# hgpeterson/nuPGCM

Measured on AMD Instinct MI355X. Metric: timesteps/sec (evolve!+invert! loop; inversion SpMV GB/s in 'roofline'), higher is better.
Workload: dtype f64 arithmetic; fp32-STORED Krylov basis and fp32 gather-layout copy of the SpMV input (the library's default at rtol >= 1e-7; products, sums, x += V y and the restart residual are fp64 - the all-fp64 figure is `fp64_basis`); 1 GPU; bowl3D_h0.02: example parameters of examples/bowl_mixing.jl (eps=0.2, alpha=1/2, mu_rho=1, N2=2, BDF2 dt=0.001), full evolve!+invert! timestep loop; tets=526720, nu=2052199, np=98592, nb=707204, nnz_A=126821881, node_block_storage=True, full_nodes=658911, surface_nodes=37733, gmres_memory=20, gmres_itmax=0, initial_guess=x_{n-1} (the reference's warm start), all_solved=True, preconditioner=Diagonal(scalar=73847.66715287707), parallelism=1 GPU

## Files before the change

### nupgcm_amd/csrc/gmres.hip

```cpp
#include <algorithm>
#include <chrono>
#include <cmath>
#include <cstdlib>
#include <type_traits>

#include <hip/hip_ext.h>

#include "common.h"
#include "spmv_device.h"
#include "spmv_window.h"

namespace npg {

constexpr int kKB = 512;
constexpr int kKP = kPartStride;
constexpr int kNS = kKB / kKP;
constexpr int kMaxG = 768;
constexpr int kMaxI = kMaxG / kNS;
constexpr int kNormSlot = kKP - 1;
constexpr int kMaxRows = 2048;

struct Snap {
    double eps, rnorm0, rnorm, beta, zeta;
    int iter, inner, done, npass, first, nreorth, pad0, pad1;
// ... 5 lines not shown
};

struct GDev {
    CsrDev A;
    const TileDesc *tile_ptr;
    int ntiles, n, mem;
    int nt_int;
    const WTileDesc *wt_ptr;
    WinDev W;
    int nwt, nwt_int, wl;
    int word;
    int wpre;
    int pkind;
    double pscalar;
    const double *pdiag;
    const double *b;
    double *x, *Vi, *w, *wt;
    double *P1, *P2, *PR;
    int G1, G2, GP1, GP2;
    int GR;
    int split;
    int64_t ldv;
    float *Vf;
    int pyth;
    int lazy2;
    int rev;
    GatherMap xg;
    const int32_t *gslot;
    int fast;
    const double *Q1, *Q2, *QR;
    int nQ1, nQ2, nQR;
    int onefold;
    int vdots;
    int fusedrows;
    struct RowsHandOff *ho;
    Snap *C, *T;
    double *c, *s, *z, *R, *hcol1, *wnorm2;
    double *hist;
    int hist_cap;
    const GParams *prm;
};

__device__ __forceinline__ void sym_givens(double a, double b, double &c, double &s, double &rho) {
    if (b == 0.0) {
        c = (a == 0.0) ? 1.0 : copysign(1.0, a);
        s = 0.0;
        rho = fabs(a);
    } else if (a == 0.0) {
        c = 0.0;
        s = copysign(1.0, b);
        rho = fabs(b);
    } else if (fabs(b) > fabs(a)) {
        const double t = a / b;
        s = copysign(1.0, b) / sqrt(1.0 + t * t);
        c = s * t;
        rho = b / s;
    } else {
        const double t = b / a;
        c = copysign(1.0, a) / sqrt(1.0 + t * t);
        s = c * t;
        rho = a / c;
    }
}

struct KShared {
    double red[kKP];
    double h[kKP], h2[kKP], cc[kKP], ss[kKP], y[kKP];
    Snap T;
    double rho, zcol;
    int fin;
    int reorth;
};

__device__ __forceinline__ void store_partial_row(double acc, double *tmp, double *part) {
    __syncthreads();
    tmp[threadIdx.x] = acc;
    __syncthreads();
    if (threadIdx.x < kKP) {
        double s = 0.0;
#pragma unroll
        for (int sl = 0; sl < kNS; ++sl) s += tmp[sl * kKP + threadIdx.x];
        part[(size_t)blockIdx.x * kKP + threadIdx.x] = s;
    }
}

__device__ void finalize_column(const GDev &d, int colj, KShared &sh, double *tmp) {
    const int t32 = threadIdx.x & (kKP - 1);
    const double h1 = d.hcol1[colj * kKP + t32];
    const double cv = d.c[t32], sv = d.s[t32];
    const Snap prev = d.T[colj];
    const double wnorm2 = d.wnorm2[colj];
    const double q1 = group_sum_dpp<kKP>(t32 <= colj ? h1 * h1 : 0.0);
    const double n2f = wnorm2 - q1;
    const bool need2 = !d.pyth && (!d.lazy2 || !(n2f >= fmax(d.prm->eta2, 1e-4) * wnorm2));
    if (need2) reduce_partials<kNS, kMaxI>(d.Q2, d.nQ2, kKP, tmp, sh.red);
    if (threadIdx.x < kKP) {
        sh.h[threadIdx.x] = h1;
        sh.h2[threadIdx.x] = (need2 && !d.fast && (int)threadIdx.x <= colj) ? sh.red[threadIdx.x] : 0.0;
        sh.cc[threadIdx.x] = cv;
        sh.ss[threadIdx.x] = sv;
    }
    __syncthreads();
    if (threadIdx.x == 0) {
        Snap t = prev;
        sh.fin = (t.done == 0) ? 1 : 0;
        sh.reorth = 0;
        if (t.done == 0) {
            double n2;
            if (d.pyth) {
                n2 = fmax(n2f, 0.0);
                if (n2f < 1e-4 * wnorm2) {
                    t.pad0 += 1;
                    t.done = 5;
                    sh.fin = 0;
                }
            } else if (!need2) {
                n2 = fmax(n2f, 0.0);
            } else {
                n2 = sh.red[kNormSlot];
            }
          if (t.done == 0) {
            const bool due = need2 && n2 < d.prm->eta2 * wnorm2;
            if (due && d.fast) t.pad1 += 1;
            const bool reorth = due && !d.fast;
            if (reorth) {
                double q = 0.0;
                for (int i = 0; i <= colj; ++i) {
// ... 199 lines not shown
            const int rb = r + kNS;
            const bool hb = rb < nr;
            const int rowa = r0 + r, rowb = r0 + (hb ? rb : r);
            double va = (k < j) ? d.Vi[vidx(rowa, k, d.n, d.ldv)] : 0.0;
            double vb = (hb && k < j) ? d.Vi[vidx(rowb, k, d.n, d.ldv)] : 0.0;
            double ta = d.wt[rowa], tb = d.wt[rowb];
            const double wa = sw[r] * inv_beta * precond_row(d, rowa);
            const double wb = hb ? sw[rb] * inv_beta * precond_row(d, rowb) : 0.0;
            if (ro) {
                ta -= group_sum_dpp<kKP>(h2k * va);
                tb -= group_sum_dpp<kKP>(h2k * vb);
            }
            if (k == j) {
                va = ta * inv_beta;
                d.Vi[vidx(rowa, j, d.n, d.ldv)] = va;
                if (hb) {
                    vb = tb * inv_beta;
                    d.Vi[vidx(rowb, j, d.n, d.ldv)] = vb;
                }
            }
            if (k == 0) {
                d.w[rowa] = wa;
                if (hb) d.w[rowb] = wb;
            }
            acc += (k == kNormSlot) ? wa * wa + wb * wb : va * wa + vb * wb;
        }
    }
    if (FUSED) store_partial_row(acc, tmp, d.P1);
}

constexpr int kRB = 256;
constexpr int kMaxRowsI = kMaxG / (kRB / 32);

template <int NG, typename BT>
__device__ __forceinline__ void load_row_cols(const BT *__restrict__ Vi, int64_t row, int64_t ldv, int j,
                                              double (&v)[8 * NG]) {
#pragma unroll
    for (int k = 0; k < 8 * NG; ++k) v[k] = (k <= j) ? (double)Vi[(size_t)k * (size_t)ldv + (size_t)row] : 0.0;
}
template <typename BT>
__device__ __forceinline__ const BT *basis_ptr(const GDev &d);
template <>
__device__ __forceinline__ const double *basis_ptr<double>(const GDev &d) { return d.Vi; }
template <>
__device__ __forceinline__ const float *basis_ptr<float>(const GDev &d) { return d.Vf; }

template <int NG>
__device__ __forceinline__ void store_partial_row_rows(const double (&acc)[8 * NG], double nrm, double *tmp, double *part) {
    const int wave = threadIdx.x >> 6, lane = threadIdx.x & 63;
    __syncthreads();
    if (lane < kKP) tmp[wave * kKP + lane] = 0.0;
    __syncthreads();
#pragma unroll
    for (int k = 0; k < 8 * NG; ++k) {
        const double s = group_sum_dpp<64>(acc[k]);
        if (lane == 0 && k < kNormSlot) tmp[wave * kKP + k] = s;
    }
    const double sn = group_sum_dpp<64>(nrm);
    if (lane == 0) tmp[wave * kKP + kNormSlot] = sn;
    __syncthreads();
    if (threadIdx.x < kKP) {
        double s = 0.0;
#pragma unroll
        for (int w = 0; w < kRB / 64; ++w) s += tmp[w * kKP + threadIdx.x];
        part[(size_t)blockIdx.x * kKP + threadIdx.x] = s;
    }
}

template <int NG>
__device__ __forceinline__ void load_row_pair_cols(const float *__restrict__ Vf, int64_t r0, bool two, int64_t ldv, int j,
                                                   float2 (&v)[8 * NG]) {
#pragma unroll
    for (int k = 0; k < 8 * NG; ++k) {
        float2 f = make_float2(0.f, 0.f);
        if (k <= j) f = *reinterpret_cast<const float2 *>(Vf + (size_t)k * (size_t)ldv + (size_t)r0);
        if (!two) f.y = 0.f;
        v[k] = f;
    }
}
template <int NG, bool VD = false>
struct RowPair {
    float2 v[8 * NG];
    double w0, w1;
    double2 t;
    int64_t r0;
    bool valid, two;
    __device__ __forceinline__ void load(const GDev &d, int64_t blk, int j) {
        r0 = 2 * (blk * kRB + threadIdx.x);
        valid = r0 < d.n;
        two = r0 + 1 < d.n;
        const int64_t rc = valid ? r0 : 0;
        load_row_pair_cols<NG>(d.Vf, rc, two, d.ldv, VD ? j - 1 : j, v);
        const double2 ww = *reinterpret_cast<const double2 *>(d.w + rc);
        if constexpr (VD) t = *reinterpret_cast<const double2 *>(d.wt + rc);
        w0 = valid ? ww.x : 0.0;
        w1 = (valid && two) ? ww.y : 0.0;
    }
};

template <int NG, typename BT, bool VD = false>
__global__ void __launch_bounds__(kRB) k_gmres_dots_rows(GDev d, int j) {
    static_assert(!VD || sizeof(BT) == 4, "the column is formed by the row-pair kernel of the fp32-stored basis");
    __shared__ double tmp[(kRB / 64) * kKP];
    double acc[8 * NG];
#pragma unroll
    for (int k = 0; k < 8 * NG; ++k) acc[k] = 0.0;
    double nrm = 0.0;
    const Snap *Tj = d.T + j;
    if (Tj->done == 0) {
        if constexpr (sizeof(BT) == 4) {
            const int64_t nblk = ((int64_t)d.n + 2 * kRB - 1) / (2 * kRB);
            RowPair<NG, VD> cur, nxt;
            int64_t blk = blockIdx.x;
            if (blk < nblk) cur.load(d, blk, j);
            double inv_beta = 0.0;
            if constexpr (VD) inv_beta = 1.0 / Tj->beta;
            for (; blk < nblk; blk += gridDim.x) {
                const bool more = blk + gridDim.x < nblk;
                if (more) nxt.load(d, blk + gridDim.x, j);
                if constexpr (VD) {
                    float2 vj = make_float2((float)(cur.t.x * inv_beta), (float)(cur.t.y * inv_beta));
                    if (cur.valid) {
                        float *col = d.Vf + (size_t)j * (size_t)d.ldv + (size_t)cur.r0;
                        if (cur.two)
                            *reinterpret_cast<float2 *>(col) = vj;
                        else
                            *col = vj.x;
                    }
                    if (!cur.two) vj.y = 0.f;
#pragma unroll
                    for (int k = 0; k < 8 * NG; ++k)
                        if (k == j) cur.v[k] = vj;
                }
#pragma unroll
                for (int k = 0; k < 8 * NG; ++k) acc[k] += (double)cur.v[k].x * cur.w0 + (double)cur.v[k].y * cur.w1;
                nrm += cur.w0 * cur.w0 + cur.w1 * cur.w1;
                if (more) cur = nxt;
            }
        } else {
            for (int64_t row = blockIdx.x * (int64_t)kRB + threadIdx.x; row < d.n; row += (int64_t)gridDim.x * kRB) {
                double v[8 * NG];
                load_row_cols<NG, BT>(basis_ptr<BT>(d), row, d.ldv, j, v);
                const double wv = d.w[row];
#pragma unroll
                for (int k = 0; k < 8 * NG; ++k) acc[k] += v[k] * wv;
                nrm += wv * wv;
            }
        }
    }
    store_partial_row_rows<NG>(acc, nrm, tmp, d.P1);
}

template <int NG, bool FAST, typename BT>
__global__ void __launch_bounds__(kRB, (NG < 4 || FAST) ? 3 : 2) k_gmres_orth_rows(GDev d, int j) {
    __shared__ double tmp[(kRB / 32) * kKP];
    __shared__ double red[kKP];
    const Snap T = d.T[j];
    if (T.done != 0) {
        if (threadIdx.x < kKP) d.P2[(size_t)blockIdx.x * kKP + threadIdx.x] = 0.0;
        return;
    }
    constexpr bool kPipe = sizeof(BT) == 4 && FAST;
    const int64_t nblk2 = ((int64_t)d.n + 2 * kRB - 1) / (2 * kRB);
    RowPair<kPipe ? NG : 1> cur;
    if constexpr (kPipe) {
        if ((int64_t)blockIdx.x < nblk2) cur.load(d, d.rev ? nblk2 - 1 - blockIdx.x : blockIdx.x, j);
    }
    reduce_partials<kRB / 32, kMaxRowsI>(d.Q1, d.nQ1, kKP, tmp, red);
    double h[8 * NG], acc[8 * NG];
#pragma unroll
    for (int k = 0; k < 8 * NG; ++k) {
        const double hv = (k <= j) ? red[k] : 0.0;
        const unsigned long long b = __double_as_longlong(hv);
        const unsigned lo = __builtin_amdgcn_readfirstlane((unsigned)b), hi = __builtin_amdgcn_readfirstlane((unsigned)(b >> 32));
        h[k] = __longlong_as_double(((unsigned long long)hi << 32) | lo);
        acc[k] = 0.0;
    }
    double nrm = 0.0;
    if (!d.onefold && blockIdx.x == 0 && threadIdx.x < kKP) {
        d.hcol1[j * kKP + threadIdx.x] = ((int)threadIdx.x <= j) ? red[threadIdx.x] : 0.0;
        if (threadIdx.x == 0) d.wnorm2[j] = red[kNormSlot];
    }
    if constexpr (kPipe) {
        const int64_t nblk = nblk2;
        RowPair<NG> nxt;
        for (int64_t blk = blockIdx.x; blk < nblk; blk += gridDim.x) {
            const int64_t nb = blk + gridDim.x;
            const bool more = nb < nblk;
            if (more) nxt.load(d, d.rev ? nblk - 1 - nb : nb, j);
            double p0 = cur.w0, p1 = cur.w1;
#pragma unroll
            for (int k = 0; k < 8 * NG; ++k) {
                p0 -= h[k] * (double)cur.v[k].x;
                p1 -= h[k] * (double)cur.v[k].y;
            }
            if (cur.valid) {
                if (cur.two)
                    *reinterpret_cast<double2 *>(d.wt + cur.r0) = make_double2(p0, p1);
                else
                    d.wt[cur.r0] = p0;
                if (d.xg.p) {
                    d.xg.p[d.xg.pos((int)cur.r0)] = (float)p0;
                    if (cur.two) d.xg.p[d.xg.pos((int)cur.r0 + 1)] = (float)p1;
                }
            } else {
                p0 = 0.0;
                p1 = 0.0;
            }
            if (!cur.two) p1 = 0.0;
            nrm += p0 * p0 + p1 * p1;
            if (more) cur = nxt;
        }
    } else if constexpr (sizeof(BT) == 4) {
        const int64_t nblk = ((int64_t)d.n + 2 * kRB - 1) / (2 * kRB);
        for (int64_t blk = blockIdx.x; blk < nblk; blk += gridDim.x) {
            const int64_t r0 = 2 * ((d.rev ? nblk - 1 - blk : blk) * kRB + threadIdx.x);
            if (r0 >= d.n) continue;
            const bool two = r0 + 1 < d.n;
            float2 v[8 * NG];
            load_row_pair_cols<NG>(d.Vf, r0, two, d.ldv, j, v);
            const double2 ww = *reinterpret_cast<const double2 *>(d.w + r0);
            double p0 = ww.x, p1 = two ? ww.y : 0.0;
#pragma unroll
            for (int k = 0; k < 8 * NG; ++k) {
                p0 -= h[k] * (double)v[k].x;
                p1 -= h[k] * (double)v[k].y;
            }
            if (two)
                *reinterpret_cast<double2 *>(d.wt + r0) = make_double2(p0, p1);
            else
                d.wt[r0] = p0;
            if (!FAST) {
#pragma unroll
// ... 34 lines not shown
            d.P2[(size_t)blockIdx.x * kKP + threadIdx.x] = t;
        }
    }
}

__global__ void __launch_bounds__(kRB) k_gmres_fold_first(GDev d, int j, double *out) {
    constexpr int NS = kRB / 32;
    __shared__ double tmp[NS * kKP];
    const int done = d.T[j].done;
    const int k = threadIdx.x & (kKP - 1), slice = threadIdx.x >> 5;
    const int nrows = d.GP1;
    double v[kMaxRowsI];
#pragma unroll
    for (int i = 0; i < kMaxRowsI; ++i) {
        const int b = slice + NS * i;
        v[i] = d.P1[(size_t)(b < nrows ? b : 0) * kKP + k];
    }
    double s = 0.0;
#pragma unroll
    for (int i = 0; i < kMaxRowsI; ++i) s += (slice + NS * i < nrows) ? v[i] : 0.0;
    tmp[slice * kKP + k] = s;
    __syncthreads();
    if (threadIdx.x < kKP && done == 0) {
        double t = 0.0;
#pragma unroll
        for (int sl = 0; sl < NS; ++sl) t += tmp[sl * kKP + threadIdx.x];
        out[threadIdx.x] = t;
        d.hcol1[j * kKP + threadIdx.x] = ((int)threadIdx.x <= j) ? t : 0.0;
        if (threadIdx.x == kNormSlot) d.wnorm2[j] = t;
    }
}

constexpr int kFusedMaxCols = 16;
constexpr int kHoLine = 16;
constexpr int kHoShards = kRB / 32;
struct RowsHandOff {
    unsigned long long gen[kHoLine];
    unsigned long long top[kHoLine];
    unsigned long long shard[kHoShards][kHoLine];
    unsigned long long status[kHoLine];
    double slice[kHoShards][kKP];
};
constexpr long long kHandOffTicks = 200000000;

template <int C> struct FusedGeom { static constexpr int B = C <= 8 ? 4 : C <= 12 ? 3 : 2, L = C <= 8 ? 2 : 1; };
static_assert(kFusedMaxCols % 4 == 0, "instances come in steps of four columns");

#define NPG_LD_AGENT(p) __hip_atomic_load((p), __ATOMIC_RELAXED, __HIP_MEMORY_SCOPE_AGENT)
#define NPG_ST_AGENT(p, v) __hip_atomic_store((p), (v), __ATOMIC_RELAXED, __HIP_MEMORY_SCOPE_AGENT)

template <int C>
struct RowTrip {
    float2 v[C];
    double w0, w1;
    template <bool VD>
    __device__ __forceinline__ void load(const GDev &d, int64_t blk, int j, double2 &t) {
        const int64_t r0 = 2 * (blk * kRB + threadIdx.x);
        const bool valid = r0 < d.n, two = r0 + 1 < d.n;
        const int64_t rc = valid ? r0 : 0;
        const int jl = VD ? j - 1 : j;
#pragma unroll
        for (int k = 0; k < C; ++k) {
            float2 f = make_float2(0.f, 0.f);
            if (k <= jl) f = *reinterpret_cast<const float2 *>(d.Vf + (size_t)k * (size_t)d.ldv + (size_t)rc);
            if (!two) f.y = 0.f;
            v[k] = f;
        }
        const double2 ww = *reinterpret_cast<const double2 *>(d.w + rc);
        if constexpr (VD) t = *reinterpret_cast<const double2 *>(d.wt + rc);
        w0 = valid ? ww.x : 0.0;
        w1 = (valid && two) ? ww.y : 0.0;
    }
};

template <int C>
__global__ void __launch_bounds__(kRB, 3) k_gmres_rows_fused(GDev d, int j) {
    constexpr int B = FusedGeom<C>::B, L = FusedGeom<C>::L;
    static_assert(kMaxG == kHoShards * kMaxRowsI && kMaxRowsI % kHoShards == 0, "a shard is one slice of the fold");
    __shared__ float2 lds_v[L * C * kRB];
    __shared__ double lds_w[L * 2 * kRB];
    __shared__ double tmp[(kRB / 32) * kKP];
    __shared__ double red[kKP];
    __shared__ int sh_role, sh_ok;
    const int tid = threadIdx.x, wave = tid >> 6, lane = tid & 63;
    const Snap *Tj = d.T + j;
    if (Tj->done != 0) {
        if (tid < kKP) {
            d.P1[(size_t)blockIdx.x * kKP + tid] = 0.0;
            d.P2[(size_t)blockIdx.x * kKP + tid] = 0.0;
        }
        return;
    }
    RowsHandOff *ho = d.ho;
    if (NPG_LD_AGENT(&ho->status[0]) != 0) return;
    unsigned long long E = 0;
    if (tid == 0) E = NPG_LD_AGENT(&ho->gen[0]);
    const int G = gridDim.x;
    const int64_t nblk = ((int64_t)d.n + 2 * kRB - 1) / (2 * kRB);
    const int nt = (int64_t)blockIdx.x < nblk ? (int)((nblk - 1 - blockIdx.x) / G) + 1 : 0;
    const int nreg = nt < B ? nt : B;
    const int nlds = nt - nreg < L ? nt - nreg : L;
    const int ne = nt - nreg - nlds;
    auto blk_of = [&](int t) { return (int64_t)blockIdx.x + (int64_t)t * G; };

    RowTrip<C> buf[B];
    double2 unused;
    double nrm = 0.0;
    {
        double acc[C];
#pragma unroll
        for (int k = 0; k < C; ++k) acc[k] = 0.0;
        double2 tq[B];
        const double inv_beta = 1.0 / Tj->beta;
#pragma unroll
        for (int s = 0; s < B - 1; ++s)
            if (s < nt) buf[s].template load<true>(d, blk_of(s), j, tq[s]);
        for (int base = 0; base < nt; base += B) {
#pragma unroll
            for (int s = 0; s < B; ++s) {
                const int t = base + s;
                if (t < nt) {
                    const int sp = (s + B - 1) % B;
                    if (t + B - 1 < nt) {
                        if (t - 1 >= ne) {
                            const int sl = t - 1 - ne;
#pragma unroll
                            for (int k = 0; k < C; ++k) lds_v[(sl * C + k) * kRB + tid] = buf[sp].v[k];
                            lds_w[(sl * 2 + 0) * kRB + tid] = buf[sp].w0;
                            lds_w[(sl * 2 + 1) * kRB + tid] = buf[sp].w1;
                        }
                        buf[sp].template load<true>(d, blk_of(t + B - 1), j, tq[sp]);
                    }
                    RowTrip<C> &cur = buf[s];
                    const int64_t r0 = 2 * (blk_of(t) * kRB + tid);
                    const bool valid = r0 < d.n, two = r0 + 1 < d.n;
                    float2 vj = make_float2((float)(tq[s].x * inv_beta), (float)(tq[s].y * inv_beta));
                    if (valid) {
                        float *col = d.Vf + (size_t)j * (size_t)d.ldv + (size_t)r0;
                        if (two)
                            *reinterpret_cast<float2 *>(col) = vj;
                        else
                            *col = vj.x;
                    }
                    if (!two) vj.y = 0.f;
#pragma unroll
                    for (int k = 0; k < C; ++k)
                        if (k == j) cur.v[k] = vj;
#pragma unroll
                    for (int k = 0; k < C; ++k) acc[k] += (double)cur.v[k].x * cur.w0 + (double)cur.v[k].y * cur.w1;
                    nrm += cur.w0 * cur.w0 + cur.w1 * cur.w1;
                }
            }
        }
        __syncthreads();
        if (lane < kKP) tmp[wave * kKP + lane] = 0.0;
        __syncthreads();
#pragma unroll
        for (int k = 0; k < C; ++k) {
            const double s = group_sum_dpp<64>(acc[k]);
            if (lane == 0) tmp[wave * kKP + k] = s;
        }
        const double sn = group_sum_dpp<64>(nrm);
        if (lane == 0) tmp[wave * kKP + kNormSlot] = sn;
        __syncthreads();
        if (tid < kKP) {
            double s = 0.0;
#pragma unroll
            for (int w = 0; w < kRB / 64; ++w) s += tmp[w * kKP + tid];
            NPG_ST_AGENT(d.P1 + (size_t)blockIdx.x * kKP + tid, s);
        }
    }

    const int shard = blockIdx.x % kHoShards;
    const int cnt = (G - shard + kHoShards - 1) / kHoShards;
    const int nsh = G < kHoShards ? G : kHoShards;
    if (wave == 0) asm volatile("s_waitcnt vmcnt(0)" ::: "memory");
    if (tid == 0) {
        const unsigned long long old = __hip_atomic_fetch_add(&ho->shard[shard][0], 1ull, __ATOMIC_RELAXED, __HIP_MEMORY_SCOPE_AGENT);
        sh_role = (old + 1 == (E + 1) * (unsigned long long)cnt) ? 1 : 0;
    }
// ... 54 lines not shown
        int ok = 1;
        const long long t0 = wall_clock64();
        while (NPG_LD_AGENT(&ho->gen[0]) < E + 1) {
            __builtin_amdgcn_s_sleep(8);
            if (wall_clock64() - t0 > kHandOffTicks) {
                NPG_ST_AGENT(&ho->status[0], 1ull);
                ok = 0;
                break;
            }
        }
        sh_ok = ok;
    }
    if (wave == 0) {
        __builtin_amdgcn_fence(__ATOMIC_ACQUIRE, "agent");
        asm volatile("s_waitcnt vmcnt(0)" ::: "memory");
    }
    __syncthreads();
    if (!sh_ok) return;
    if (tid < kKP) {
        const unsigned long long bits = NPG_LD_AGENT(reinterpret_cast<const unsigned long long *>(d.Q1) + tid);
        red[tid] = __longlong_as_double(bits);
    }
    __syncthreads();

    double h[C];
#pragma unroll
    for (int k = 0; k < C; ++k) {
        const double hv = (k <= j) ? red[k] : 0.0;
        const unsigned long long b = __double_as_longlong(hv);
        const unsigned lo = __builtin_amdgcn_readfirstlane((unsigned)b), hi = __builtin_amdgcn_readfirstlane((unsigned)(b >> 32));
        h[k] = __longlong_as_double(((unsigned long long)hi << 32) | lo);
    }
    nrm = 0.0;
    auto update = [&](const RowTrip<C> &cur, int t) {
        const int64_t r0 = 2 * (blk_of(t) * kRB + tid);
        const bool valid = r0 < d.n, two = r0 + 1 < d.n;
        double p0 = cur.w0, p1 = cur.w1;
#pragma unroll
        for (int k = 0; k < C; ++k) {
            float vx = cur.v[k].x, vy = cur.v[k].y;
            asm("" : "+v"(vx), "+v"(vy));
            p0 -= h[k] * (double)vx;
            p1 -= h[k] * (double)vy;
        }
        if (valid) {
            if (two)
                *reinterpret_cast<double2 *>(d.wt + r0) = make_double2(p0, p1);
            else
                d.wt[r0] = p0;
            if (d.xg.p) {
                d.xg.p[d.xg.pos((int)r0)] = (float)p0;
                if (two) d.xg.p[d.xg.pos((int)r0 + 1)] = (float)p1;
            }
        } else {
            p0 = 0.0;
            p1 = 0.0;
        }
        if (!two) p1 = 0.0;
        nrm += p0 * p0 + p1 * p1;
    };
    for (int t = 0; t < ne; ++t) {
        update(early, t);
        if (t + 1 < ne) early.template load<false>(d, blk_of(t + 1), j, unused);
    }
#pragma unroll
    for (int sl = 0; sl < L; ++sl) {
        if (sl < nlds) {
#pragma unroll
            for (int k = 0; k < C; ++k) early.v[k] = lds_v[(sl * C + k) * kRB + tid];
            early.w0 = lds_w[(sl * 2 + 0) * kRB + tid];
            early.w1 = lds_w[(sl * 2 + 1) * kRB + tid];
            update(early, ne + sl);
        }
    }
    {
        const int tr = nt - nreg, rot = tr % B;
#pragma unroll
        for (int ro = 0; ro < B; ++ro) {
            if (ro == rot) {
#pragma unroll
                for (int r = 0; r < B; ++r)
                    if (r < nreg) update(buf[(ro + r) % B], tr + r);
            }
        }
    }
    const double sn2 = group_sum_dpp<64>(nrm);
    __syncthreads();
    if (lane == 0) tmp[wave] = sn2;
    __syncthreads();
    if (tid < kKP) {
        double tt = 0.0;
        if (tid == kNormSlot)
            for (int w = 0; w < kRB / 64; ++w) tt += tmp[w];
        d.P2[(size_t)blockIdx.x * kKP + tid] = tt;
    }
}

__global__ void __launch_bounds__(kKB, 6) k_gmres_orth(GDev d, int j) {
    __shared__ KShared sh;
    __shared__ double tmp[kNS * kKP];
    const Snap T = d.T[j];
    reduce_partials<kNS, kMaxI>(d.Q1, d.nQ1, kKP, tmp, sh.red);
    if (T.done != 0) return;
    const int k = threadIdx.x & (kKP - 1), slot = threadIdx.x >> 5;
    if (blockIdx.x == 0 && threadIdx.x < kKP) {
        d.hcol1[j * kKP + threadIdx.x] = ((int)threadIdx.x <= j) ? sh.red[threadIdx.x] : 0.0;
        if (threadIdx.x == 0) d.wnorm2[j] = sh.red[kNormSlot];
    }
    const double hk = (k <= j) ? sh.red[k] : 0.0;
    double acc = 0.0;
    const int64_t stride = (int64_t)gridDim.x * kNS;
    for (int64_t row = (int64_t)blockIdx.x * kNS + slot; row < d.n; row += 2 * stride) {
        const int64_t rowb = row + stride;
        const bool hb = rowb < d.n;
        const double va = (k <= j) ? d.Vi[vidx(row, k, d.n, d.ldv)] : 0.0;
        const double vb = (hb && k <= j) ? d.Vi[vidx(rowb, k, d.n, d.ldv)] : 0.0;
        const double wa = d.w[row];
// ... 126 lines not shown
    double *P1 = nullptr, *P2 = nullptr, *PR = nullptr;
    Snap *C = nullptr, *T = nullptr;
    double *c = nullptr, *s = nullptr, *z = nullptr, *R = nullptr, *hcol1 = nullptr, *wnorm2 = nullptr;
    double *hist = nullptr;
    int hist_cap = 0;
    GParams *prm = nullptr;
    Snap *h_C = nullptr;
    GParams *h_prm = nullptr;
    int64_t hist_len = 0;
    hipGraph_t graph[2] = {nullptr, nullptr};
    hipGraphExec_t exec[2] = {nullptr, nullptr};
    hipEvent_t ev[2] = {nullptr, nullptr};
    GDev key;
    bool have_graph = false;
    bool profile = false;
    bool explicit_norm = false;
    bool safe_mode = false;
    int split_mode = -1;
    int basis_bits = 0;
    int halo_overlap = -1;
    int dist_graph = -1;
    std::vector<hipEvent_t> pev;
    double prof_ms = 0.0;
    int64_t prof_launches = 0;
    int gather32 = -1;
    float *xg = nullptr;
    int64_t xg_len = 0;
    int xg_key[3] = {-1, -1, -1};
    npg_halo *halo = nullptr;
    double *Rg = nullptr;
    int64_t n_ghost = 0;
    RowsHandOff *ho = nullptr;
    unsigned long long *h_ho = nullptr;
    int fused_blocks = -1;
    bool fused_off = false;
    int32_t cfg[kCfgLen] = {};
    bool have_cfg = false;
};

static int fold_rows(npg_gmres *ws, const double *part, int nrows, int slot, hipStream_t st, bool dist) {
    double *out = ws->Rg + slot * kKP;
    if (dist) return fold_allreduce_rows(ws->ctx, part, nrows, out, st);
    hipLaunchKernelGGL(k_reduce_rows, dim3(1), dim3(1024), 0, st, part, nrows, out);
    return NPG_OK;
}

template <int NG, typename BT>
static void launch_rows_bt(const GDev &d, int j, hipStream_t st, bool orth) {
    if (orth && d.fast)
        hipLaunchKernelGGL((k_gmres_orth_rows<NG, true, BT>), dim3(d.GR), dim3(kRB), 0, st, d, j);
    else if (orth)
        hipLaunchKernelGGL((k_gmres_orth_rows<NG, false, BT>), dim3(d.GR), dim3(kRB), 0, st, d, j);
    else
        hipLaunchKernelGGL((k_gmres_dots_rows<NG, BT>), dim3(d.GR), dim3(kRB), 0, st, d, j);
}
template <int NG>
static void launch_rows(const GDev &d, int j, hipStream_t st, bool orth) {
    if (d.Vf && d.vdots && !orth)
        hipLaunchKernelGGL((k_gmres_dots_rows<NG, float, true>), dim3(d.GR), dim3(kRB), 0, st, d, j);
    else if (d.Vf)
        launch_rows_bt<NG, float>(d, j, st, orth);
    else
        launch_rows_bt<NG, double>(d, j, st, orth);
}

static void launch_rows_kernel(const GDev &d, int j, hipStream_t st, bool orth) {
// ... 349 lines not shown
        const int64_t nbr = A->block_rows(), need = 4 * nslots + (A->n - nbr) + 8;
        if (ws->xg_len < need) {
            if (ws->xg) NPG_HIP(hipFree(ws->xg));
            ws->xg = nullptr;
            NPG_HIP(hipMalloc((void **)&ws->xg, (size_t)need * sizeof(float)));
            ws->xg_len = need;
            ws->xg_key[0] = -1;
        }
        if (ws->xg_key[0] != A->nfull || ws->xg_key[1] != A->nsurf || ws->xg_key[2] != (int)A->n) {
            NPG_HIP(hipMemsetAsync(ws->xg, 0, (size_t)ws->xg_len * sizeof(float), st));
            ws->xg_key[0] = A->nfull;
            ws->xg_key[1] = A->nsurf;
            ws->xg_key[2] = (int)A->n;
        }
        d.xg = GatherMap{ws->xg, 3 * A->nfull, A->nfull, (int)nbr, (int)(4 * nslots - nbr)};
        d.gslot = A->wtile_ptr ? A->gslot : nullptr;
        static const int win_env = getenv("NPG_GMRES_WINDOW") ? atoi(getenv("NPG_GMRES_WINDOW")) : 1;
        if (win_env && ws->gather32 != 2 && d.split && A->wtile_ptr && !A->pk9 && nbr > 0) {
            d.wt_ptr = A->wtile_ptr;
            d.W = win_view(A);
            d.nwt = A->nwtiles;
            d.nwt_int = A->nwtiles_interior;
            d.wl = A->wlanes;
            static const int ord_env = getenv("NPG_WIN_ORD") ? atoi(getenv("NPG_WIN_ORD")) : 0;
            static const int pre_env = getenv("NPG_WIN_PRE") ? atoi(getenv("NPG_WIN_PRE")) : 1;
            d.word = ord_env || (A->nwrow_tiles == 0 && A->m > A->block_rows());
            d.wpre = pre_env;
        }
    }
    const char *onefold_env = getenv("NPG_GMRES_ONEFOLD");
    d.onefold = (!dist && d.split && d.fast && !(onefold_env && atoi(onefold_env) == 0)) ? 1 : 0;
    d.vdots = (d.onefold && d.Vf) ? 1 : 0;
    const char *fusedrows_env = getenv("NPG_GMRES_FUSEDROWS");
    if (!dist && d.split && d.fast && d.Vf && !d.rev && !ws->fused_off && !(fusedrows_env && atoi(fusedrows_env) == 0)) {
        if (ws->fused_blocks < 0) ws->fused_blocks = rows_fused_blocks_per_cu();
        if (d.GR <= ctx->num_cu * ws->fused_blocks) {
            if (!ws->ho) {
                NPG_HIP(hipMalloc((void **)&ws->ho, sizeof(RowsHandOff)));
                NPG_HIP(hipMemsetAsync(ws->ho, 0, sizeof(RowsHandOff), st));
                NPG_HIP(hipHostMalloc((void **)&ws->h_ho, 2 * sizeof(unsigned long long), hipHostMallocDefault));
                ws->h_ho[0] = ws->h_ho[1] = 0;
            }
            d.fusedrows = 1;
            d.ho = ws->ho;
            d.onefold = d.vdots = 1;
        }
    }
    if (dist) {
        d.Q1 = ws->Rg;
        d.Q2 = ws->Rg + kKP;
        d.QR = ws->Rg + 2 * kKP;
        d.nQ1 = d.nQ2 = d.nQR = 1;
    } else {
        d.Q1 = d.P1;
        d.Q2 = d.P2;
        d.QR = d.PR;
        d.nQ1 = d.GP1;
        d.nQ2 = d.GP2;
        d.nQR = d.G1;
        if (d.onefold) {
            d.Q1 = ws->Rg;
            d.nQ1 = 1;
        }
    }
    d.C = ws->C;
    d.T = ws->T;
    d.c = ws->c;
    d.s = ws->s;
    d.z = ws->z;
    d.R = ws->R;
    d.hcol1 = ws->hcol1;
    d.wnorm2 = ws->wnorm2;
    d.hist = ws->hist;
    d.hist_cap = ws->hist_cap;
    d.prm = ws->prm;

    if (itmax <= 0) itmax = 2 * ws->n;
    ws->h_prm->atol = atol;
    ws->h_prm->rtol = rtol;
// ... 5 lines not shown
    c0.first = 1;
    ws->h_C[0] = c0;
    NPG_HIP(hipMemcpyAsync(ws->C, ws->h_C, sizeof(Snap), hipMemcpyHostToDevice, st));
    NPG_HIP(hipStreamSynchronize(st));

    static const int traced = getenv("ROCPROFILER_LIBRARY_CTOR") || getenv("ROCPROF_OUTPUT_PATH") || getenv("ROCP_TOOL_LIBRARIES");
    static const int eager = getenv("NPG_GMRES_EAGER") ? atoi(getenv("NPG_GMRES_EAGER")) : traced;
    static bool said = false;
    if (eager && traced && !getenv("NPG_GMRES_EAGER") && !said && (said = true))
        fprintf(stderr, "[npg] rocprofv3 detected: GMRES restart cycles are launched eagerly instead of replayed from hipGraphs "
                        "(rocprofiler-sdk faults on graph launches that wrap the AQL ring; NPG_GMRES_EAGER=0 overrides)\n");
    static const int trace = getenv("NPG_GMRES_TRACE") ? atoi(getenv("NPG_GMRES_TRACE")) : 0;

    static const int dist_graph_env = getenv("NPG_DIST_GRAPH") ? atoi(getenv("NPG_DIST_GRAPH")) : -1;
    const bool kernel_only = dist && comm_is_kernel_only(ws->ctx);
    const bool graph_dist = dist && !ws->ctx->shm &&
                            (kernel_only ? (dist_graph_env != 0 && ws->dist_graph != 0) : ((ws->dist_graph > 0 || dist_graph_env > 0) && ws->ctx->comm));
    auto capture_graphs = [&]() -> int {
        for (int k = 0; k < 2; ++k) {
            if (ws->exec[k]) hipGraphExecDestroy(ws->exec[k]);
            if (ws->graph[k]) hipGraphDestroy(ws->graph[k]);
            ws->exec[k] = nullptr;
            ws->graph[k] = nullptr;
            ws->have_graph = false;
            NPG_HIP(hipStreamBeginCapture(st, hipStreamCaptureModeThreadLocal));
            int rcg = launch_cycle(d, A->lanes, st, nullptr, ws, dist != nullptr);
            if (rcg) {
                hipGraph_t broken = nullptr;
                hipStreamEndCapture(st, &broken);
                if (broken) hipGraphDestroy(broken);
                return rcg;
            }
            NPG_HIP(hipMemcpyAsync(ws->h_C + k, ws->C, sizeof(Snap), hipMemcpyDeviceToHost, st));
            if (d.fusedrows) NPG_HIP(hipMemcpyAsync(ws->h_ho + k, d.ho->status, sizeof(unsigned long long), hipMemcpyDeviceToHost, st));
            NPG_HIP(hipStreamEndCapture(st, &ws->graph[k]));
            NPG_HIP(hipGraphInstantiate(&ws->exec[k], ws->graph[k], nullptr, nullptr, 0));
        }
        memcpy(&ws->key, &d, sizeof d);
        ws->have_graph = true;
        return NPG_OK;
    };
    const bool use_graph = (!dist || graph_dist) && !eager && !ws->profile;
    if (use_graph && (!ws->have_graph || memcmp(&ws->key, &d, sizeof(GDev)) != 0)) {
        int rcg = capture_graphs();
        if (rcg) return rcg;
    }

    if (dist) {
        int rcd = halo_exchange_raw(ws->halo, d.x);
        if (rcd) return rcd;
    }
    launch_residual(d, A->lanes, st);
    NPG_HIP(hipGetLastError());
    if (dist) {
        int rcd = fold_rows(ws, d.PR, d.G1, 2, st, true);
        if (rcd) return rcd;
    }
    const int64_t max_cycles = (itmax + ws->mem - 1) / ws->mem + 1;
    Snap last{};
    double t_launch = 0.0;
    int64_t n_launch = 0;
    auto enqueue_cycle = [&](int slot) -> int {
        const auto l0 = std::chrono::steady_clock::now();
        if (eager || (dist && !graph_dist)) {
            int rcc = launch_cycle(d, A->lanes, st, nullptr, ws, dist != nullptr);
            if (rcc) return rcc;
            NPG_HIP(hipMemcpyAsync(ws->h_C + slot, ws->C, sizeof(Snap), hipMemcpyDeviceToHost, st));
            if (d.fusedrows) NPG_HIP(hipMemcpyAsync(ws->h_ho + slot, d.ho->status, sizeof(unsigned long long), hipMemcpyDeviceToHost, st));
        } else {
            NPG_HIP(hipGraphLaunch(ws->exec[slot], st));
        }
        NPG_HIP(hipEventRecord(ws->ev[slot], st));
        t_launch += std::chrono::duration<double>(std::chrono::steady_clock::now() - l0).count();
        ++n_launch;
        return NPG_OK;
    };
    auto fused_gave_up = [&]() -> int {
        hipStreamSynchronize(st);
        hipMemset(ws->ho, 0, sizeof(RowsHandOff));
        ws->h_ho[0] = ws->h_ho[1] = 0;
        ws->fused_off = true;
        ws->have_graph = false;
        npg::set_error("npg_gmres_solve: the grid-wide hand-off of the fused row kernel timed out (a workgroup was not resident); "
                       "the iterate is not valid - this workspace uses the separate row launches from now on");
        return NPG_EHIP;
    };
    if (!ws->profile) {
        int rc0 = enqueue_cycle(0);
        if (rc0) return rc0;
        for (int64_t cyc = 0;; ++cyc) {
            const int cur = (int)(cyc & 1), nxt = cur ^ 1;
            const bool more = cyc + 1 < max_cycles;
            if (more) {
                rc0 = enqueue_cycle(nxt);
                if (rc0) return rc0;
            }
            NPG_HIP(hipEventSynchronize(ws->ev[cur]));
            last = ws->h_C[cur];
            if (d.fusedrows && ws->h_ho[cur] != 0) return fused_gave_up();
            if (last.done == 5) {
                NPG_HIP(hipStreamSynchronize(st));
                d.pyth = 0;
                ws->explicit_norm = true;
                if (use_graph) {
                    rc0 = capture_graphs();
                    if (rc0) return rc0;
                }
                last.done = 0;
                last.inner = 0;
                ws->h_C[cur] = last;
                NPG_HIP(hipMemcpyAsync(ws->C, ws->h_C + cur, sizeof(Snap), hipMemcpyHostToDevice, st));
                if (dist && (rc0 = halo_exchange_raw(ws->halo, d.x))) return rc0;
                launch_residual(d, A->lanes, st);
                if (dist && (rc0 = fold_rows(ws, d.PR, d.G1, 2, st, true))) return rc0;
                NPG_HIP(hipStreamSynchronize(st));
                rc0 = enqueue_cycle(cur);
                if (rc0) return rc0;
                cyc = -1 + (cur == 0 ? 0 : 1);
                continue;
            }
            if (last.done != 0 || !more) break;
        }
        NPG_HIP(hipStreamSynchronize(st));
        if (trace)
            fprintf(stderr,
                    "[npg gmres] %s: %lld cycle launches, %.1f us host time per launch, %d iterations, %.1f us wall per "
                    "iteration, %d second GS passes, fused rows %d (row grid %d, %d workgroups per CU admitted)\n",
                    eager ? "eager" : "graph", (long long)n_launch, 1e6 * t_launch / (double)n_launch, last.iter,
                    1e6 * std::chrono::duration<double>(std::chrono::steady_clock::now() - t0).count() /
                        std::max(1, last.iter),
                    last.nreorth, d.fusedrows, d.GR, ws->fused_blocks);
    } else {
        if (ws->pev.empty()) {
            ws->pev.resize(2 * ws->mem);
            for (auto &e : ws->pev) NPG_HIP(hipEventCreate(&e));
        }
        for (int64_t cyc = 0; cyc < max_cycles; ++cyc) {
            int rcp = launch_cycle(d, A->lanes, st, ws->pev.data(), ws, dist != nullptr);
            if (rcp) return rcp;
            NPG_HIP(hipMemcpyAsync(ws->h_C, ws->C, sizeof(Snap), hipMemcpyDeviceToHost, st));
            if (d.fusedrows) NPG_HIP(hipMemcpyAsync(ws->h_ho, d.ho->status, sizeof(unsigned long long), hipMemcpyDeviceToHost, st));
            NPG_HIP(hipStreamSynchronize(st));
            if (d.fusedrows && ws->h_ho[0] != 0) return fused_gave_up();
            last = ws->h_C[0];
            if (last.done == 5) {
                d.pyth = 0;
                ws->explicit_norm = true;
                last.done = 0;
                last.inner = 0;
                ws->h_C[0] = last;
                NPG_HIP(hipMemcpyAsync(ws->C, ws->h_C, sizeof(Snap), hipMemcpyHostToDevice, st));
                int rcx = NPG_OK;
                if (dist && (rcx = halo_exchange_raw(ws->halo, d.x))) return rcx;
                launch_residual(d, A->lanes, st);
                if (dist && (rcx = fold_rows(ws, d.PR, d.G1, 2, st, true))) return rcx;
                NPG_HIP(hipStreamSynchronize(st));
                continue;
            }
            if (last.done != 0) break;
            for (int j = 0; j < ws->mem; ++j) {
                float ms = 0.f;
                NPG_HIP(hipEventElapsedTime(&ms, ws->pev[2 * j], ws->pev[2 * j + 1]));
                ws->prof_ms += ms;
                ws->prof_launches += 1;
            }
        }
    }
    ws->hist_len = std::min<int64_t>((int64_t)last.iter + 1, ws->hist_cap);
    {
        const int a_nt = d.wt_ptr ? d.nwt : d.ntiles;
        const int32_t cfg[kCfgLen] = {d.split, d.Vf ? 32 : 64, d.fast, d.xg.p ? (d.xg.nbr == 0 ? 2 : 1) : 0, d.wt_ptr ? 1 : 0,
                                      d.wt_ptr ? d.wl : 0, d.wt_ptr ? d.word : 0, A->lanes, A->pk9 ? 1 : 0, dist ? 1 : 0, d.pyth,
                                      a_nt, d.split ? std::min(d.G1, std::max(1, a_nt)) : d.G1, d.split ? d.GR : d.G2, d.n, d.mem,
                                      d.lazy2, d.fusedrows};
// ... 79 lines not shown
```

Before: 0.7032 timesteps/s.

## Form next Krylov basis column inside the Gram-Schmidt update kernel

The row update kernel now computes the next column's norm from the already-reduced dots (Pythagorean estimate). When no second Gram-Schmidt pass is needed, it writes the normalized fp32 basis column j+1 directly and skips the fp64 wt write. The following dots kernel then reads a ready flag and skips re-reading wt and rewriting the column, saving one full-vector read and write per iteration. The cost is extra hand-off state, a per-column readiness flag, and a slightly more complex control path with fallback counting.

```diff
diff --git a/nupgcm_amd/csrc/gmres.hip b/nupgcm_amd/csrc/gmres.hip
--- a/nupgcm_amd/csrc/gmres.hip
+++ b/nupgcm_amd/csrc/gmres.hip
@@ -61,6 +61,7 @@
     int nQ1, nQ2, nQR;
     int onefold;
     int vdots;
+    int nextcol;
     int fusedrows;
     struct RowsHandOff *ho;
     Snap *C, *T;
@@ -113,15 +114,26 @@
     }
 }
 
+struct NextNorm {
+    double n2f;
+    bool need2;
+};
+__device__ __forceinline__ NextNorm next_norm(const GDev &d, int colj, int t32, double h1, double wnorm2) {
+    const double q1 = group_sum_dpp<kKP>(t32 <= colj ? h1 * h1 : 0.0);
+    const double n2f = wnorm2 - q1;
+    const bool need2 = !d.pyth && (!d.lazy2 || !(n2f >= fmax(d.prm->eta2, 1e-4) * wnorm2));
+    return NextNorm{n2f, need2};
+}
+
 __device__ void finalize_column(const GDev &d, int colj, KShared &sh, double *tmp) {
     const int t32 = threadIdx.x & (kKP - 1);
     const double h1 = d.hcol1[colj * kKP + t32];
     const double cv = d.c[t32], sv = d.s[t32];
     const Snap prev = d.T[colj];
     const double wnorm2 = d.wnorm2[colj];
-    const double q1 = group_sum_dpp<kKP>(t32 <= colj ? h1 * h1 : 0.0);
-    const double n2f = wnorm2 - q1;
-    const bool need2 = !d.pyth && (!d.lazy2 || !(n2f >= fmax(d.prm->eta2, 1e-4) * wnorm2));
+    const NextNorm nn = next_norm(d, colj, t32, h1, wnorm2);
+    const double n2f = nn.n2f;
+    const bool need2 = nn.need2;
     if (need2) reduce_partials<kNS, kMaxI>(d.Q2, d.nQ2, kKP, tmp, sh.red);
     if (threadIdx.x < kKP) {
         sh.h[threadIdx.x] = h1;
@@ -387,6 +399,41 @@
 constexpr int kRB = 256;
 constexpr int kMaxRowsI = kMaxG / (kRB / 32);
 
+constexpr int kHoLine = 16;
+constexpr int kHoShards = kRB / 32;
+constexpr int kHoCopy = 3;
+struct RowsHandOff {
+    unsigned long long gen[kHoLine];
+    unsigned long long top[kHoLine];
+    unsigned long long shard[kHoShards][kHoLine];
+    unsigned long long status[kHoLine];
+    double slice[kHoShards][kKP];
+    int colready[kKP + 1];
+};
+
+struct NextCol {
+    int formed, skip;
+    double inv_beta;
+};
+__device__ __forceinline__ NextCol next_col(const GDev &d, int j, const double *red) {
+    NextCol nc{0, 0, 0.0};
+    if (!d.nextcol) return nc;
+    const int t32 = threadIdx.x & (kKP - 1);
+    const NextNorm nn = next_norm(d, j, t32, red[t32], red[kNormSlot]);
+    const double beta = sqrt(fmax(nn.n2f, 0.0));
+    const double ib = 1.0 / beta;
+    nc.formed = __builtin_amdgcn_readfirstlane((!nn.need2 && beta > 0.0) ? 1 : 0);
+    nc.skip = (nc.formed && j + 1 == d.mem) ? 1 : 0;
+    const unsigned long long b = __double_as_longlong(ib);
+    const unsigned lo = __builtin_amdgcn_readfirstlane((unsigned)b), hi = __builtin_amdgcn_readfirstlane((unsigned)(b >> 32));
+    nc.inv_beta = __longlong_as_double(((unsigned long long)hi << 32) | lo);
+    if (blockIdx.x == 0 && threadIdx.x == 0) {
+        d.ho->colready[j + 1] = nc.formed;
+        d.ho->status[nc.formed ? 1 : 2] += 1;
+    }
+    return nc;
+}
+
 template <int NG, typename BT>
 __device__ __forceinline__ void load_row_cols(const BT *__restrict__ Vi, int64_t row, int64_t ldv, int j,
                                               double (&v)[8 * NG]) {
@@ -440,14 +487,16 @@
     double2 t;
     int64_t r0;
     bool valid, two;
-    __device__ __forceinline__ void load(const GDev &d, int64_t blk, int j) {
+    __device__ __forceinline__ void load(const GDev &d, int64_t blk, int j, bool ready = false) {
         r0 = 2 * (blk * kRB + threadIdx.x);
         valid = r0 < d.n;
         two = r0 + 1 < d.n;
         const int64_t rc = valid ? r0 : 0;
-        load_row_pair_cols<NG>(d.Vf, rc, two, d.ldv, VD ? j - 1 : j, v);
+        load_row_pair_cols<NG>(d.Vf, rc, two, d.ldv, (VD && !ready) ? j - 1 : j, v);
         const double2 ww = *reinterpret_cast<const double2 *>(d.w + rc);
-        if constexpr (VD) t = *reinterpret_cast<const double2 *>(d.wt + rc);
+        if constexpr (VD) {
+            if (!ready) t = *reinterpret_cast<const double2 *>(d.wt + rc);
+        }
         w0 = valid ? ww.x : 0.0;
         w1 = (valid && two) ? ww.y : 0.0;
     }
@@ -467,13 +516,15 @@
             const int64_t nblk = ((int64_t)d.n + 2 * kRB - 1) / (2 * kRB);
             RowPair<NG, VD> cur, nxt;
             int64_t blk = blockIdx.x;
-            if (blk < nblk) cur.load(d, blk, j);
+            bool ready = false;
+            if constexpr (VD) ready = d.nextcol && j > 0 && __builtin_amdgcn_readfirstlane(d.ho->colready[j]) != 0;
+            if (blk < nblk) cur.load(d, blk, j, ready);
             double inv_beta = 0.0;
             if constexpr (VD) inv_beta = 1.0 / Tj->beta;
             for (; blk < nblk; blk += gridDim.x) {
                 const bool more = blk + gridDim.x < nblk;
-                if (more) nxt.load(d, blk + gridDim.x, j);
-                if constexpr (VD) {
+                if (more) nxt.load(d, blk + gridDim.x, j, ready);
+                if (VD && !ready) {
                     float2 vj = make_float2((float)(cur.t.x * inv_beta), (float)(cur.t.y * inv_beta));
                     if (cur.valid) {
                         float *col = d.Vf + (size_t)j * (size_t)d.ldv + (size_t)cur.r0;
@@ -518,8 +569,9 @@
     constexpr bool kPipe = sizeof(BT) == 4 && FAST;
     const int64_t nblk2 = ((int64_t)d.n + 2 * kRB - 1) / (2 * kRB);
     RowPair<kPipe ? NG : 1> cur;
+    const bool late = kPipe && d.nextcol && j + 1 == d.mem;
     if constexpr (kPipe) {
-        if ((int64_t)blockIdx.x < nblk2) cur.load(d, d.rev ? nblk2 - 1 - blockIdx.x : blockIdx.x, j);
+        if (!late && (int64_t)blockIdx.x < nblk2) cur.load(d, d.rev ? nblk2 - 1 - blockIdx.x : blockIdx.x, j);
     }
     reduce_partials<kRB / 32, kMaxRowsI>(d.Q1, d.nQ1, kKP, tmp, red);
     double h[8 * NG], acc[8 * NG];
@@ -537,7 +589,10 @@
         if (threadIdx.x == 0) d.wnorm2[j] = red[kNormSlot];
     }
     if constexpr (kPipe) {
-        const int64_t nblk = nblk2;
+        const NextCol nc = next_col(d, j, red);
+        const bool keep_wt = !nc.formed || !d.xg.p;
+        const int64_t nblk = nc.skip ? 0 : nblk2;
+        if (late && !nc.skip && (int64_t)blockIdx.x < nblk) cur.load(d, d.rev ? nblk - 1 - blockIdx.x : blockIdx.x, j);
         RowPair<NG> nxt;
         for (int64_t blk = blockIdx.x; blk < nblk; blk += gridDim.x) {
             const int64_t nb = blk + gridDim.x;
@@ -550,10 +605,19 @@
                 p1 -= h[k] * (double)cur.v[k].y;
             }
             if (cur.valid) {
-                if (cur.two)
-                    *reinterpret_cast<double2 *>(d.wt + cur.r0) = make_double2(p0, p1);
-                else
-                    d.wt[cur.r0] = p0;
+                if (keep_wt) {
+                    if (cur.two)
+                        *reinterpret_cast<double2 *>(d.wt + cur.r0) = make_double2(p0, p1);
+                    else
+                        d.wt[cur.r0] = p0;
+                }
+                if (nc.formed) {
+                    float *col = d.Vf + (size_t)(j + 1) * (size_t)d.ldv + (size_t)cur.r0;
+                    if (cur.two)
+                        *reinterpret_cast<float2 *>(col) = make_float2((float)(p0 * nc.inv_beta), (float)(p1 * nc.inv_beta));
+                    else
+                        *col = (float)(p0 * nc.inv_beta);
+                }
                 if (d.xg.p) {
                     d.xg.p[d.xg.pos((int)cur.r0)] = (float)p0;
                     if (cur.two) d.xg.p[d.xg.pos((int)cur.r0 + 1)] = (float)p1;
@@ -654,15 +718,6 @@
 }
 
 constexpr int kFusedMaxCols = 16;
-constexpr int kHoLine = 16;
-constexpr int kHoShards = kRB / 32;
-struct RowsHandOff {
-    unsigned long long gen[kHoLine];
-    unsigned long long top[kHoLine];
-    unsigned long long shard[kHoShards][kHoLine];
-    unsigned long long status[kHoLine];
-    double slice[kHoShards][kKP];
-};
 constexpr long long kHandOffTicks = 200000000;
 
 template <int C> struct FusedGeom { static constexpr int B = C <= 8 ? 4 : C <= 12 ? 3 : 2, L = C <= 8 ? 2 : 1; };
@@ -676,11 +731,11 @@
     float2 v[C];
     double w0, w1;
     template <bool VD>
-    __device__ __forceinline__ void load(const GDev &d, int64_t blk, int j, double2 &t) {
+    __device__ __forceinline__ void load(const GDev &d, int64_t blk, int j, double2 &t, bool ready = false) {
         const int64_t r0 = 2 * (blk * kRB + threadIdx.x);
         const bool valid = r0 < d.n, two = r0 + 1 < d.n;
         const int64_t rc = valid ? r0 : 0;
-        const int jl = VD ? j - 1 : j;
+        const int jl = (VD && !ready) ? j - 1 : j;
 #pragma unroll
         for (int k = 0; k < C; ++k) {
             float2 f = make_float2(0.f, 0.f);
@@ -689,7 +744,9 @@
             v[k] = f;
         }
         const double2 ww = *reinterpret_cast<const double2 *>(d.w + rc);
-        if constexpr (VD) t = *reinterpret_cast<const double2 *>(d.wt + rc);
+        if constexpr (VD) {
+            if (!ready) t = *reinterpret_cast<const double2 *>(d.wt + rc);
+        }
         w0 = valid ? ww.x : 0.0;
         w1 = (valid && two) ? ww.y : 0.0;
     }
@@ -734,9 +791,10 @@
         for (int k = 0; k < C; ++k) acc[k] = 0.0;
         double2 tq[B];
         const double inv_beta = 1.0 / Tj->beta;
+        const bool ready = d.nextcol && j > 0 && __builtin_amdgcn_readfirstlane(ho->colready[j]) != 0;
 #pragma unroll
         for (int s = 0; s < B - 1; ++s)
-            if (s < nt) buf[s].template load<true>(d, blk_of(s), j, tq[s]);
+            if (s < nt) buf[s].template load<true>(d, blk_of(s), j, tq[s], ready);
         for (int base = 0; base < nt; base += B) {
 #pragma unroll
             for (int s = 0; s < B; ++s) {
@@ -751,23 +809,25 @@
                             lds_w[(sl * 2 + 0) * kRB + tid] = buf[sp].w0;
                             lds_w[(sl * 2 + 1) * kRB + tid] = buf[sp].w1;
                         }
-                        buf[sp].template load<true>(d, blk_of(t + B - 1), j, tq[sp]);
+                        buf[sp].template load<true>(d, blk_of(t + B - 1), j, tq[sp], ready);
                     }
                     RowTrip<C> &cur = buf[s];
-                    const int64_t r0 = 2 * (blk_of(t) * kRB + tid);
-                    const bool valid = r0 < d.n, two = r0 + 1 < d.n;
-                    float2 vj = make_float2((float)(tq[s].x * inv_beta), (float)(tq[s].y * inv_beta));
-                    if (valid) {
-                        float *col = d.Vf + (size_t)j * (size_t)d.ldv + (size_t)r0;
-                        if (two)
-                            *reinterpret_cast<float2 *>(col) = vj;
-                        else
-                            *col = vj.x;
+                    if (!ready) {
+                        const int64_t r0 = 2 * (blk_of(t) * kRB + tid);
+                        const bool valid = r0 < d.n, two = r0 + 1 < d.n;
+                        float2 vj = make_float2((float)(tq[s].x * inv_beta), (float)(tq[s].y * inv_beta));
+                        if (valid) {
+                            float *col = d.Vf + (size_t)j * (size_t)d.ldv + (size_t)r0;
+                            if (two)
+                                *reinterpret_cast<float2 *>(col) = vj;
+                            else
+                                *col = vj.x;
+                        }
+                        if (!two) vj.y = 0.f;
+#pragma unroll
+                        for (int k = 0; k < C; ++k)
+                            if (k == j) cur.v[k] = vj;
                     }
-                    if (!two) vj.y = 0.f;
-#pragma unroll
-                    for (int k = 0; k < C; ++k)
-                        if (k == j) cur.v[k] = vj;
 #pragma unroll
                     for (int k = 0; k < C; ++k) acc[k] += (double)cur.v[k].x * cur.w0 + (double)cur.v[k].y * cur.w1;
                     nrm += cur.w0 * cur.w0 + cur.w1 * cur.w1;
@@ -888,6 +948,8 @@
         h[k] = __longlong_as_double(((unsigned long long)hi << 32) | lo);
     }
     nrm = 0.0;
+    const NextCol nc = next_col(d, j, red);
+    const bool keep_wt = !nc.formed || !d.xg.p;
     auto update = [&](const RowTrip<C> &cur, int t) {
         const int64_t r0 = 2 * (blk_of(t) * kRB + tid);
         const bool valid = r0 < d.n, two = r0 + 1 < d.n;
@@ -900,10 +962,19 @@
             p1 -= h[k] * (double)vy;
         }
         if (valid) {
-            if (two)
-                *reinterpret_cast<double2 *>(d.wt + r0) = make_double2(p0, p1);
-            else
-                d.wt[r0] = p0;
+            if (keep_wt) {
+                if (two)
+                    *reinterpret_cast<double2 *>(d.wt + r0) = make_double2(p0, p1);
+                else
+                    d.wt[r0] = p0;
+            }
+            if (nc.formed) {
+                float *col = d.Vf + (size_t)(j + 1) * (size_t)d.ldv + (size_t)r0;
+                if (two)
+                    *reinterpret_cast<float2 *>(col) = make_float2((float)(p0 * nc.inv_beta), (float)(p1 * nc.inv_beta));
+                else
+                    *col = (float)(p0 * nc.inv_beta);
+            }
             if (d.xg.p) {
                 d.xg.p[d.xg.pos((int)r0)] = (float)p0;
                 if (two) d.xg.p[d.xg.pos((int)r0 + 1)] = (float)p1;
@@ -915,6 +986,7 @@
         if (!two) p1 = 0.0;
         nrm += p0 * p0 + p1 * p1;
     };
+    if (!nc.skip) {
     for (int t = 0; t < ne; ++t) {
         update(early, t);
         if (t + 1 < ne) early.template load<false>(d, blk_of(t + 1), j, unused);
@@ -939,6 +1011,7 @@
                     if (r < nreg) update(buf[(ro + r) % B], tr + r);
             }
         }
+    }
     }
     const double sn2 = group_sum_dpp<64>(nrm);
     __syncthreads();
@@ -1131,6 +1204,7 @@
     int64_t n_ghost = 0;
     RowsHandOff *ho = nullptr;
     unsigned long long *h_ho = nullptr;
+    unsigned long long nc_base[2] = {0, 0};
     int fused_blocks = -1;
     bool fused_off = false;
     int32_t cfg[kCfgLen] = {};
@@ -1546,19 +1620,30 @@
     d.onefold = (!dist && d.split && d.fast && !(onefold_env && atoi(onefold_env) == 0)) ? 1 : 0;
     d.vdots = (d.onefold && d.Vf) ? 1 : 0;
     const char *fusedrows_env = getenv("NPG_GMRES_FUSEDROWS");
+    auto alloc_handoff = [&]() -> int {
+        if (!ws->ho) {
+            NPG_HIP(hipMalloc((void **)&ws->ho, sizeof(RowsHandOff)));
+            NPG_HIP(hipMemsetAsync(ws->ho, 0, sizeof(RowsHandOff), st));
+            NPG_HIP(hipHostMalloc((void **)&ws->h_ho, 2 * kHoCopy * sizeof(unsigned long long), hipHostMallocDefault));
+            memset(ws->h_ho, 0, 2 * kHoCopy * sizeof(unsigned long long));
+            ws->nc_base[0] = ws->nc_base[1] = 0;
+        }
+        return NPG_OK;
+    };
     if (!dist && d.split && d.fast && d.Vf && !d.rev && !ws->fused_off && !(fusedrows_env && atoi(fusedrows_env) == 0)) {
         if (ws->fused_blocks < 0) ws->fused_blocks = rows_fused_blocks_per_cu();
         if (d.GR <= ctx->num_cu * ws->fused_blocks) {
-            if (!ws->ho) {
-                NPG_HIP(hipMalloc((void **)&ws->ho, sizeof(RowsHandOff)));
-                NPG_HIP(hipMemsetAsync(ws->ho, 0, sizeof(RowsHandOff), st));
-                NPG_HIP(hipHostMalloc((void **)&ws->h_ho, 2 * sizeof(unsigned long long), hipHostMallocDefault));
-                ws->h_ho[0] = ws->h_ho[1] = 0;
-            }
+            if (int rch = alloc_handoff()) return rch;
             d.fusedrows = 1;
             d.ho = ws->ho;
             d.onefold = d.vdots = 1;
         }
+    }
+    const char *nextcol_env = getenv("NPG_GMRES_NEXTCOL");
+    if (d.vdots && !(nextcol_env && atoi(nextcol_env) == 0)) {
+        if (int rch = alloc_handoff()) return rch;
+        d.nextcol = 1;
+        d.ho = ws->ho;
     }
     if (dist) {
         d.Q1 = ws->Rg;
@@ -1630,7 +1715,7 @@
                 return rcg;
             }
             NPG_HIP(hipMemcpyAsync(ws->h_C + k, ws->C, sizeof(Snap), hipMemcpyDeviceToHost, st));
-            if (d.fusedrows) NPG_HIP(hipMemcpyAsync(ws->h_ho + k, d.ho->status, sizeof(unsigned long long), hipMemcpyDeviceToHost, st));
+            if (d.fusedrows) NPG_HIP(hipMemcpyAsync(ws->h_ho + kHoCopy * k, d.ho->status, kHoCopy * sizeof(unsigned long long), hipMemcpyDeviceToHost, st));
             NPG_HIP(hipStreamEndCapture(st, &ws->graph[k]));
             NPG_HIP(hipGraphInstantiate(&ws->exec[k], ws->graph[k], nullptr, nullptr, 0));
         }
@@ -1664,7 +1749,7 @@
             int rcc = launch_cycle(d, A->lanes, st, nullptr, ws, dist != nullptr);
             if (rcc) return rcc;
             NPG_HIP(hipMemcpyAsync(ws->h_C + slot, ws->C, sizeof(Snap), hipMemcpyDeviceToHost, st));
-            if (d.fusedrows) NPG_HIP(hipMemcpyAsync(ws->h_ho + slot, d.ho->status, sizeof(unsigned long long), hipMemcpyDeviceToHost, st));
+            if (d.fusedrows) NPG_HIP(hipMemcpyAsync(ws->h_ho + kHoCopy * slot, d.ho->status, kHoCopy * sizeof(unsigned long long), hipMemcpyDeviceToHost, st));
         } else {
             NPG_HIP(hipGraphLaunch(ws->exec[slot], st));
         }
@@ -1676,7 +1761,8 @@
     auto fused_gave_up = [&]() -> int {
         hipStreamSynchronize(st);
         hipMemset(ws->ho, 0, sizeof(RowsHandOff));
-        ws->h_ho[0] = ws->h_ho[1] = 0;
+        memset(ws->h_ho, 0, 2 * kHoCopy * sizeof(unsigned long long));
+        ws->nc_base[0] = ws->nc_base[1] = 0;
         ws->fused_off = true;
         ws->have_graph = false;
         npg::set_error("npg_gmres_solve: the grid-wide hand-off of the fused row kernel timed out (a workgroup was not resident); "
@@ -1695,7 +1781,7 @@
             }
             NPG_HIP(hipEventSynchronize(ws->ev[cur]));
             last = ws->h_C[cur];
-            if (d.fusedrows && ws->h_ho[cur] != 0) return fused_gave_up();
+            if (d.fusedrows && ws->h_ho[kHoCopy * cur] != 0) return fused_gave_up();
             if (last.done == 5) {
                 NPG_HIP(hipStreamSynchronize(st));
                 d.pyth = 0;
@@ -1720,14 +1806,28 @@
             if (last.done != 0 || !more) break;
         }
         NPG_HIP(hipStreamSynchronize(st));
-        if (trace)
+        if (trace) {
+            unsigned long long nc[2] = {0, 0};
+            if (d.nextcol) {
+                const unsigned long long *src = ws->h_ho + kHoCopy * (int)((n_launch - 1) & 1);
+                if (!d.fusedrows) {
+                    NPG_HIP(hipMemcpy(ws->h_ho, d.ho->status, kHoCopy * sizeof(unsigned long long), hipMemcpyDeviceToHost));
+                    src = ws->h_ho;
+                }
+                for (int q = 0; q < 2; ++q) {
+                    nc[q] = src[1 + q] - ws->nc_base[q];
+                    ws->nc_base[q] = src[1 + q];
+                }
+            }
             fprintf(stderr,
                     "[npg gmres] %s: %lld cycle launches, %.1f us host time per launch, %d iterations, %.1f us wall per "
-                    "iteration, %d second GS passes, fused rows %d (row grid %d, %d workgroups per CU admitted)\n",
+                    "iteration, %d second GS passes, fused rows %d (row grid %d, %d workgroups per CU admitted), next column %d "
+                    "(%llu formed by an update, %llu fell back)\n",
                     eager ? "eager" : "graph", (long long)n_launch, 1e6 * t_launch / (double)n_launch, last.iter,
                     1e6 * std::chrono::duration<double>(std::chrono::steady_clock::now() - t0).count() /
                         std::max(1, last.iter),
-                    last.nreorth, d.fusedrows, d.GR, ws->fused_blocks);
+                    last.nreorth, d.fusedrows, d.GR, ws->fused_blocks, d.nextcol, nc[0], nc[1]);
+        }
     } else {
         if (ws->pev.empty()) {
             ws->pev.resize(2 * ws->mem);
@@ -1737,7 +1837,7 @@
             int rcp = launch_cycle(d, A->lanes, st, ws->pev.data(), ws, dist != nullptr);
             if (rcp) return rcp;
             NPG_HIP(hipMemcpyAsync(ws->h_C, ws->C, sizeof(Snap), hipMemcpyDeviceToHost, st));
-            if (d.fusedrows) NPG_HIP(hipMemcpyAsync(ws->h_ho, d.ho->status, sizeof(unsigned long long), hipMemcpyDeviceToHost, st));
+            if (d.fusedrows) NPG_HIP(hipMemcpyAsync(ws->h_ho, d.ho->status, kHoCopy * sizeof(unsigned long long), hipMemcpyDeviceToHost, st));
             NPG_HIP(hipStreamSynchronize(st));
             if (d.fusedrows && ws->h_ho[0] != 0) return fused_gave_up();
             last = ws->h_C[0];
```

After: 0.7132 timesteps/s (median of 6 runs). About the same (+1.4%).
